# magneano/shyft

Hardware: AMD Instinct MI355X
Metric: cell-steps/sec (cells×timesteps/wall) for pt_gs_k at 1/2/4/8 MI355X (higher is better)
Workload: dtype f64

## Files before the change

shyft_amd/csrc/device/gamma_lean.h:

```cpp
#pragma once
#include <hip/hip_runtime.h>

#include "special.h"

namespace shyft_dev {

__device__ __forceinline__ double exp_fast(double x, const gsb_k& k) {
    double r = gsb_exp(x, k);
    if (!(__builtin_fabs(x) <= 708.0)) r = dexp(x);
    return r;
}
__device__ __forceinline__ double log_fast(double x, const gsb_k& k) {
    double r = gsb_log(x, k);
    if (!(x >= 2.2250738585072014e-308 && x <= 1.7976931348623157e308)) r = dlog(x);
    return r;
}

__device__ __forceinline__ gamma_p_result gsb_gamma_pq(double a, double x, double lga, double eps, double ap1,
                                                       const gsb_k& k, bool& ok) {
    const double lx = gsb_log(x, k);
    const double arg = a * lx - x - lga;
    ok = a > 0.0 && x >= 2.2250738585072014e-308 && x <= 1.7976931348623157e308 && __builtin_fabs(arg) <= 708.0;
    const double prefix = gsb_exp(arg, k);
    gamma_p_result r;
    r.prefix = prefix;
    r.p = r.p1 = 0.0;
    if (!ok) return r;
    if (x < ap1) {
        double ap = a, E = 1.0, B = 0.0, xn = 1.0;
        for (int n = 1; n <= 2000; ++n) {
            ap = ap + 1.0;
            xn = xn * x;
            E = E * ap;
            B = __builtin_fma(B, ap, xn);
            if (xn < eps * (B + E)) break;
        }
        ok = ok && E <= detmath::GPQ_SCALE_HI;
        const double aE = a * E;
        const double pp = prefix * ((B + E) / aE);
        const double pp1 = prefix * (B / aE);
        r.p = pp < 1.0 ? pp : 1.0;
        r.p1 = pp1 < 1.0 ? pp1 : 1.0;
    } else {
        double bcf = x + 1.0 - a;
        double Pm = 1.0, Qm = 0.0, P = bcf, Qd = 1.0, di = 0.0, bigP = 0.0;
        for (int i = 1; i <= 2000; ++i) {
            di = di + 1.0;
            const double an = -di * (di - a);
            bcf = bcf + 2.0;
            const double Pn = __builtin_fma(bcf, P, an * Pm);
            const double Qn = __builtin_fma(bcf, Qd, an * Qm);
            const double cross = Pn * Qd;
            const double diff = cross - P * Qn;
            Pm = P; Qm = Qd;
            P = Pn; Qd = Qn;
            if (__builtin_fabs(diff) <= eps * __builtin_fabs(cross)) break;
            bigP = __builtin_fmax(bigP, __builtin_fabs(P));
        }
        ok = ok && !(bigP > detmath::GPQ_SCALE_HI);
        const double q = prefix * (Qd / P);
        const double q1 = q + prefix / a;
        const double pp = 1.0 - q;
        const double pp1 = 1.0 - q1;
        r.p = pp > 0.0 ? pp : 0.0;
        r.p1 = pp1 > 0.0 ? pp1 : 0.0;
    }
    return r;
}

__device__ __noinline__ gamma_p_result gs_gamma_pq_general(double a, double x, double lga) {
    return gamma_p_prefix(a, x, lga, detmath::gamma_snow_policy_eps(a));
}

}
```

shyft_amd/csrc/device/ptgsk_dev.h:

```cpp
#pragma once
#include <hip/hip_runtime.h>
#include <stdint.h>

#include "pt_dev.h"
#include "special.h"
#include "gamma_lean.h"
#include "../include_internal/layout.h"


namespace shyft_dev {

constexpr double GS_TOL = 1.0e-10;

struct gs_state {
    double albedo, lwc, surface_heat, alpha, sdc_melt_mean, acc_melt, iso_pot_energy, temp_swe;
};

struct lgamma_cache {
    double a = -1.0, v = 0.0;
    __device__ inline double get(double shape) {
        if (shape != a) { a = shape; v = dlgamma(shape); }
        return v;
    }
    __device__ inline double job_lgamma(double shape) { return get(shape); }
};
template <bool DEFER_JOB = false>
struct lgamma_cache_lds {
    double* a;
    double* v;
    __device__ inline double get(double shape) {
        const int t = threadIdx.x;
        if (shape != a[t]) { a[t] = shape; v[t] = dlgamma(shape); }
        return v[t];
    }
    __device__ inline double job_lgamma(double shape) {
        if (!DEFER_JOB) return get(shape);
        a[threadIdx.x] = shape;
        return __builtin_nan("");
    }
};

struct gs_lw {
    double p = __builtin_nan(""), p1 = __builtin_nan("");
};

__device__ __forceinline__ gamma_p_result gs_gamma_pq_cs(double a, double x, double lga) {
    const gsb_k k = gsb_load();
    bool ok;
    gamma_p_result r = gsb_gamma_pq(a, x, lga, detmath::gamma_snow_policy_eps(a), a + 1.0, k, ok);
    if (!ok) r = gs_gamma_pq_general(a, x, lga);
    return r;
}

template <class LGC>
__device__ inline void calc_snow_state(double shape, double scale, double y0, double lambda, double lwd,
                                       double max_water_frac, double temp_swe, double& swe, double& sca,
                                       LGC& lgc, gs_lw& lw) {
    lw.p = lw.p1 = __builtin_nan("");
    double y = 0.0, y1 = 0.0;
    const double m = shape * scale;
    if (lambda <= 0.0) {
        swe = m;
        sca = 1.0 - y0;
    } else if (lambda / scale > 1.3 * shape + 20.0) {
        swe = sca = 0.0;
        return;
    } else {
        const double x = lambda / scale;
        const gamma_p_result g = gs_gamma_pq_cs(shape, x, lgc.get(shape));
        y = g.p;
        y1 = y - g.prefix / shape;
        swe = m * (1.0 - y1) - lambda * (1 - y);
        sca = (1.0 - y) * (1.0 - y0);
    }
    if (lwd > m)
        swe *= 1.0 + max_water_frac;
    else if (lwd > 0.0) {
        const double sat = lwd / max_water_frac;
        const double x = sat / scale;
        const gamma_p_result g = gs_gamma_pq_cs(shape, x, lgc.get(shape));
        lw.p = g.p;
        lw.p1 = g.p1;
        const double ssa = g.p;
        const double ssa1 = ssa - g.prefix / shape;
        const double liqwat = max_water_frac * (m * (ssa1 - y1) + sat * (1.0 - ssa) - lambda * (1.0 - y));
        swe += liqwat;
    }
    swe += temp_swe;
    swe *= 1.0 - y0;
}

__device__ inline double gs_calc_q(double a, double b, double z, double lga) {
    const gamma_p_result g = gs_gamma_pq(a, z / b, lga);
    return a * b * g.p1 + z * (1.0 - g.p);
}


#ifdef SHYFT_PROF
#define SHYFT_PROF_NF , int& nf_evals
#else
#define SHYFT_PROF_NF
#endif
__device__ __noinline__ double gs_corr_lwc(double z1, double a1, double b1, double a2, double b2,
                                           double q1, double lga2 SHYFT_PROF_NF) {
#ifdef SHYFT_ABLATE_BRENT
    return z1 * 0.5;
#endif
    const double Q1 = q1 == q1 ? q1 : gs_calc_q(a1, b1, z1, dlgamma(a1));
    auto f = [&](double z) {
#ifdef SHYFT_PROF
        ++nf_evals;
#endif
        const double v = gs_calc_q(a2, b2, z, lga2) - Q1;
        return v * v;
    };
    double min = 0.0, max = z1;
    const double tolerance = 0x1p-11;
    const double golden = (double)0.3819660f;
    double x, w, v, u, delta, delta2, fu, fv, fw, fx, mid, fract1, fract2;
    x = w = v = max;
    fw = fv = fx = f(x);
    delta2 = delta = 0;
    int count = 60;
    do {
        mid = (min + max) / 2;
        fract1 = tolerance * fabs(x) + tolerance / 4;
        fract2 = 2 * fract1;
        if (fabs(x - mid) <= (fract2 - (max - min) / 2)) break;
        if (fabs(delta2) > fract1) {
            double r = (x - w) * (fx - fv);
            double q = (x - v) * (fx - fw);
            double p = (x - v) * q - (x - w) * r;
            q = 2 * (q - r);
            if (q > 0) p = -p;
            q = fabs(q);
            double td = delta2;
            delta2 = delta;
            if ((fabs(p) >= fabs(q * td / 2)) || (p <= q * (min - x)) || (p >= q * (max - x))) {
                delta2 = (x >= mid) ? min - x : max - x;
                delta = golden * delta2;
            } else {
                delta = p / q;
                u = x + delta;
                if (((u - min) < fract2) || ((max - u) < fract2)) delta = (mid - x) < 0 ? -fabs(fract1) : fabs(fract1);
            }
        } else {
            delta2 = (x >= mid) ? min - x : max - x;
            delta = golden * delta2;
        }
        u = (fabs(delta) >= fract1) ? (x + delta) : (delta > 0 ? x + fabs(fract1) : x - fabs(fract1));
        fu = f(u);
        if (fu <= fx) {
            if (u >= x) min = x; else max = x;
            v = w; w = x; x = u;
            fv = fw; fw = fx; fx = fu;
        } else {
            if (u < x) min = u; else max = u;
            if ((fu <= fw) || (w == x)) {
                v = w; w = u; fv = fw; fw = fu;
            } else if ((fu <= fv) || (v == x) || (v == w)) {
                v = u; fv = fu;
            }
        }
    } while (--count);
    return x;
}

struct gs_cell {
    double forest_fraction, altitude;
    double cv2;
    double inv_cv2;
};

struct gs_mid {
    bool done;
    bool need;
    double snow, rain, potential_melt, start_storage, sdc_scale;
};

struct gs_carry {
    double storage = 0.0;
    gs_lw lw;
    bool ok = false;
};

template <class LGC, class Enqueue, class NewShape>
__device__ inline void gs_front(gs_state& s, gs_mid& m, bool start_melt, double dt_s, double dt_us,
                                      const double* __restrict__ P, const gs_cell& cc, double T, double rad,
                                      double prec_mm_h, double wind_speed, double rel_hum, LGC& lgc,
                                      const gs_carry& carry, Enqueue&& enqueue, NewShape&& new_shape) {
    m.need = false;
    m.done = false;
    double sdc_melt_mean = s.sdc_melt_mean;
    double acc_melt = s.acc_melt;
    double iso_pot_energy = s.iso_pot_energy;
    const double prec = (prec_mm_h * dt_us) / 3600000000.0;
    if (start_melt) acc_melt = iso_pot_energy = 0.0;
    double snow, rain;
    if (T < P[PK_TX]) { snow = prec; rain = 0.0; }
    else { snow = 0.0; rain = prec; }
    if (snow < GS_TOL && sdc_melt_mean < GS_TOL && acc_melt < 0.0) {
        m.done = true;
        return;
    }
    double albedo = s.albedo;
    double lwc = s.lwc;
    double surface_heat = s.surface_heat;
    double alpha = s.alpha;
    const double temp_swe = s.temp_swe;
    double sca = 0.0, storage = 0.0;
    const double min_albedo = P[PK_MIN_ALBEDO];
    const double max_albedo = P[PK_MAX_ALBEDO];
    const double ibgf = P[PK_IBGF];
    const double max_water = P[PK_MAX_WATER];

    const double T_k = T + 273.15;
    const double turb = P[PK_WIND_SCALE] * wind_speed + P[PK_WIND_CONST];
    double vapour_pressure = 33.864 * (dpow8(7.38e-3 * T + 0.8072) - 1.9e-5 * fabs(1.8 * T + 48.0) + 1.316e-3) * rel_hum;
    if (T < 0.0) vapour_pressure *= 1.0 + 9.72e-3 * T + 4.2e-5 * T * T;

    if (snow > GS_TOL)
        albedo += snow * P[PK_ALBEDO_RANGE] / P[PK_SNOWFALL_RESET];
    else {
        if (T < 0.0) albedo -= P[PK_SLOW_DECAY];
        else albedo = min_albedo + P[PK_FAST_DECAY] * (albedo - min_albedo);
    }
    albedo = smax(smin(albedo, max_albedo), min_albedo);

    const double sigma = 5.670373e-8;
    double effect = rad * (1.0 - albedo);
    const dexp_pair gse = dexp2(6.87e-2 * dlog(vapour_pressure / T_k), 0.103 * T - 0.186);
    effect += 0.98 * sigma * gse.a * dpow4(T_k);
    if (T > 0.0 && snow < GS_TOL) effect += rain * T * 4180.0 / dt_s;
    if (T <= 0.0 && rain < GS_TOL) effect += snow * T * 2050.0 / dt_s;

    if (P[PK_ISO] != 0.0) {
        const double iso_effect = effect - P[PK_BB0] + turb * (T + 1.7 * (vapour_pressure - 6.12));
        iso_pot_energy += iso_effect * dt_s / 333660.0;
    }
    const double sst = smin(0.0, 1.16 * T - 2.09);
    if (sst > -GS_TOL)
        effect += turb * (T + 1.7 * (vapour_pressure - 6.12)) - P[PK_BB0];
    else
        effect += turb * (T - sst + 1.7 * (vapour_pressure - 6.132 * gse.b)) -
                  0.98 * sigma * dpow4(sst + 273.15);

    double delta_sh = -surface_heat;
    surface_heat = P[PK_SURFACE_MAG] * 2050.0 * sst * 0.5;
    delta_sh += surface_heat;
    double energy = effect * dt_s;
    if (delta_sh > 0.0) energy -= delta_sh;
    const double potential_melt = smax(0.0, energy / 333660.0);

    double sdc_scale = sdc_melt_mean / alpha;
    gs_lw lw;
    if (carry.ok && !start_melt) {
        storage = carry.storage;
        lw = carry.lw;
    } else {
        calc_snow_state(alpha, sdc_scale, ibgf, acc_melt, lwc, max_water, temp_swe, storage, sca, lgc, lw);
    }
    m.start_storage = storage;

    if (acc_melt < 0.0) {
        if (snow < GS_TOL) snow = 0.0;
        else {
            const double alpha_prev = alpha;
            const double sdc_scale_prev = sdc_scale;
            const double sdc_snow = snow / (1.0 - ibgf);
            alpha = (sdc_melt_mean * alpha + sdc_snow / cc.cv2) / (sdc_snow + sdc_melt_mean);
            sdc_melt_mean += sdc_snow;
            sdc_scale = sdc_melt_mean / alpha;
            if (lwc > 0.0 && sdc_snow > 0.01 * sdc_melt_mean) {
                m.need = true;
                const double z1 = lwc / max_water;
                const double a1 = alpha_prev;
                const double b1 = sdc_scale_prev > 0.0 ? sdc_scale_prev : sdc_scale;
                const double q1 = (sdc_scale_prev > 0.0 && lw.p == lw.p) ? a1 * b1 * lw.p1 + z1 * (1.0 - lw.p)
                                                                          : __builtin_nan("");
                enqueue(z1, a1, b1, alpha, sdc_scale, q1, lgc.job_lgamma(alpha));
            }
        }
        if (!(sdc_melt_mean <= potential_melt)) {
            double lwc_end = lwc + rain;
            double shape = alpha;
            if (potential_melt > 0.0) {
                lwc_end += potential_melt;
                shape = smax(0.1, (sdc_melt_mean - potential_melt) / sdc_scale);
                if (shape > cc.inv_cv2) shape = cc.inv_cv2;
            }
            if (m.need || lwc_end > 0.0) new_shape(shape);
        }
    }
    (void)sca;
    m.snow = snow;
    m.rain = rain;
    m.potential_melt = potential_melt;
    m.sdc_scale = sdc_scale;
    s.albedo = albedo;
    s.surface_heat = surface_heat;
    s.iso_pot_energy = iso_pot_energy;
    s.alpha = alpha;
    s.sdc_melt_mean = sdc_melt_mean;
    s.acc_melt = acc_melt;
}

template <class LGC, class Enqueue>
__device__ inline void gs_front(gs_state& s, gs_mid& m, bool start_melt, double dt_s, double dt_us,
                                      const double* __restrict__ P, const gs_cell& cc, double T, double rad,
                                      double prec_mm_h, double wind_speed, double rel_hum, LGC& lgc,
                                      const gs_carry& carry, Enqueue&& enqueue) {
    gs_front(s, m, start_melt, dt_s, dt_us, P, cc, T, rad, prec_mm_h, wind_speed, rel_hum, lgc, carry, enqueue,
             [](double) {});
}

template <class LGC>
__device__ inline void gs_back(gs_state& s, const gs_mid& m, double z, double& r_sca, double& r_storage,
                                     double& r_outflow, bool snow_season, double dt_us, const double* __restrict__ P,
                                     const gs_cell& cc, double prec_mm_h, LGC& lgc, gs_carry& carry) {
    if (m.done) {
        carry.ok = false;
        carry.storage = 0.0;
        carry.lw = gs_lw();
        s.albedo = P[PK_MAX_ALBEDO];
        s.surface_heat = 0.0;
        s.iso_pot_energy = 0.0;
        r_sca = 0.0;
        r_storage = 0.0;
        r_outflow = prec_mm_h;
        return;
    }
    const double ibgf = P[PK_IBGF];
    const double max_water = P[PK_MAX_WATER];
    const double prec = (prec_mm_h * dt_us) / 3600000000.0;
    double snow = m.snow;
    const double rain = m.rain;
    double lwc = s.lwc, alpha = s.alpha, temp_swe = s.temp_swe, sca = 0.0;
    double storage = m.start_storage;
    double sdc_melt_mean = s.sdc_melt_mean, acc_melt = s.acc_melt, potential_melt = m.potential_melt;
    double sdc_scale = m.sdc_scale;
    if (acc_melt < 0.0) {
        if (m.need) lwc = z * max_water;
        lwc += rain;
        if (sdc_melt_mean <= potential_melt) {
            storage = 0.0;
            sca = sdc_melt_mean = 0.0;
            alpha = P[PK_INV_CV2_PARAM];
            temp_swe = lwc = 0.0;
            acc_melt = -1.0;
            sdc_scale = 0.0;
        } else if (potential_melt > 0.0) {
            sdc_melt_mean -= potential_melt;
            lwc += potential_melt;
            alpha = smax(0.1, sdc_melt_mean / sdc_scale);
            if (alpha > cc.inv_cv2) alpha = cc.inv_cv2;
            sdc_scale = sdc_melt_mean / alpha;
        }
    } else {
        temp_swe += snow / (1.0 - ibgf);
        if (temp_swe > 0.0) {
            const double melt = smin(temp_swe, potential_melt);
            temp_swe -= melt;
            potential_melt -= melt;
            lwc += melt;
            if (temp_swe < GS_TOL) temp_swe = 0.0;
        }
        acc_melt += potential_melt;
        lwc += rain + potential_melt;
        if (P[PK_ISO] == 0.0 || snow_season) {
            if (storage < smax(0.2, 2 * temp_swe) || storage < 0.2 * rain) {
                storage += snow;
                if (storage > GS_TOL) {
                    sca = 1.0 - ibgf;
                    sdc_melt_mean = storage / sca;
                } else {
                    sca = sdc_melt_mean = 0.0;
                }
                alpha = P[PK_INV_CV2_PARAM];
                temp_swe = lwc = 0.0;
                acc_melt = -1.0;
                sdc_scale = sdc_melt_mean / alpha;
            }
        }
    }
    calc_snow_state(alpha, sdc_scale, ibgf, acc_melt, lwc, max_water, temp_swe, storage, sca, lgc, carry.lw);
    carry.storage = storage;
    carry.ok = true;
    double outflow = prec + m.start_storage - storage;
    if (outflow < 0.0) outflow = 0.0;

    s.lwc = lwc;
    s.alpha = alpha;
    s.sdc_melt_mean = sdc_melt_mean;
    s.acc_melt = acc_melt;
    s.temp_swe = temp_swe;
    r_sca = sca;
    r_storage = storage;
    r_outflow = (outflow * 3600000000.0) / dt_us;
}

__device__ inline double kirchner_f(double ln_q, double p_minus_e, double c1, double c2, double c3) {
    const dexp_pair ge = dexp2(c1 + c2 * ln_q + c3 * ln_q * ln_q, -ln_q);
    return ge.a >= 1.e-30 ? ge.a * (p_minus_e * ge.b - 1.0) : 0.0;
}

template <bool INL = false>
__device__ inline bool kirchner_step(double& q, double& q_avg, double p, double e, double t1, double c1, double c2,
                                     double c3) {
    const double abs_err = 1.0e-7, rel_err = 1.0e-8;
    if (q < 0.00001) q = 0.00001;
#ifdef SHYFT_ABLATE_KIRCHNER
    q_avg = q; q = q + 0.01 * (p - e); return true;
#endif
    const double pe = p - e;
    const kmath<INL> km;
    auto kirchner_f = [&](double ln_q, double p_minus_e, double c1_, double c2_, double c3_) {
        const dexp_pair ge = km.exp2(c1_ + c2_ * ln_q + c3_ * ln_q * ln_q, -ln_q);
        return ge.a >= 1.e-30 ? ge.a * (p_minus_e * ge.b - 1.0) : 0.0;
    };
    auto dexp = [&](double v) { return km.exp(v); };
    auto dlog = [&](double v) { return km.log(v); };
    double x = dlog(q);
    double dxdt = kirchner_f(x, pe, c1, c2, c3);
    double t = 0.0, dt = t1;
    double x_old = x, dxdt_old = dxdt, t_old = 0.0;
    double k3 = 0, k4 = 0, k5 = 0, k6 = 0;
    double area = 0.0, f_a = q, t_a = 0.0;
    int attempts = 0;
    bool ok = true;
    const double b21 = 1.0 / 5;
    const double b31 = 3.0 / 40, b32 = 9.0 / 40;
    const double b41 = 44.0 / 45, b42 = -56.0 / 15, b43 = 32.0 / 9;
    const double b51 = 19372.0 / 6561, b52 = -25360.0 / 2187, b53 = 64448.0 / 6561, b54 = -212.0 / 729;
    const double b61 = 9017.0 / 3168, b62 = -355.0 / 33, b63 = 46732.0 / 5247, b64 = 49.0 / 176, b65 = -5103.0 / 18656;
    const double c1_ = 35.0 / 384, c3_ = 500.0 / 1113, c4_ = 125.0 / 192, c5_ = -2187.0 / 6784, c6_ = 11.0 / 84;
    const double dc1 = c1_ - 5179.0 / 57600, dc3 = c3_ - 7571.0 / 16695, dc4 = c4_ - 393.0 / 640,
                 dc5 = c5_ - -92097.0 / 339200, dc6 = c6_ - 187.0 / 2100, dc7 = -1.0 / 40;
    auto attempt = [&](const double h) -> bool {
        double xt = 1.0 * x + h * b21 * dxdt;
        const double k2 = kirchner_f(xt, pe, c1, c2, c3);
        xt = 1.0 * x + h * b31 * dxdt + h * b32 * k2;
        const double s3 = kirchner_f(xt, pe, c1, c2, c3);
        xt = 1.0 * x + h * b41 * dxdt + h * b42 * k2 + h * b43 * s3;
        const double s4 = kirchner_f(xt, pe, c1, c2, c3);
        xt = 1.0 * x + h * b51 * dxdt + h * b52 * k2 + h * b53 * s3 + h * b54 * s4;
        const double s5 = kirchner_f(xt, pe, c1, c2, c3);
        xt = 1.0 * x + h * b61 * dxdt + h * b62 * k2 + h * b63 * s3 + h * b64 * s4 + h * b65 * s5;
        const double s6 = kirchner_f(xt, pe, c1, c2, c3);
        const double xo = 1.0 * x + h * c1_ * dxdt + h * c3_ * s3 + h * c4_ * s4 + h * c5_ * s5 + h * c6_ * s6;
        const double dxdt_o = kirchner_f(xo, pe, c1, c2, c3);
        const double xerr = h * dc1 * dxdt + h * dc3 * s3 + h * dc4 * s4 + h * dc5 * s5 + h * dc6 * s6 + h * dc7 * dxdt_o;
        const double err = fabs(xerr) / (abs_err + rel_err * (1.0 * fabs(x) + 1.0 * h * fabs(dxdt)));
        if (err > 1.0) {
            dt = h * smax(0.9 * dexp(-1.0 / 3.0 * dlog(err)), 1.0 / 5.0);
            return ++attempts < 500;
        }
        attempts = 0;
        t_old = t;
        t = t + h;
        dt = h;
        if (err < 0.5 && t < t1) {
            const double e2 = smax(0.00032, err);
            dt = h * (9.0 / 10.0 * dexp(-1.0 / 5.0 * dlog(e2)));
        }
        x_old = x; dxdt_old = dxdt;
        x = xo; dxdt = dxdt_o;
        k3 = s3; k4 = s4; k5 = s5; k6 = s6;
        if (t < t1) {
            const double fv = dexp(x);
            area += 0.5 * (f_a + fv) * (t - t_a);
            f_a = fv;
            t_a = t;
// ... 48 lines not shown
```

shyft_amd/csrc/kernels/ptgsk.hip:

```cpp
#include <hip/hip_runtime.h>
#include <stdint.h>
#include <stdlib.h>

#include "../device/ptgsk_dev.h"
#include "../device/gs_brent.h"
#include "../device/stream.h"
#include "../device/wave_place.h"
#include "../include_internal/kernels.h"
#include "../../../include/shyft_hip.h"

using namespace shyft_dev;

#define GS_BRENT_JOB gs_corr_lwc_lean

#ifdef SHYFT_PROF
__device__ unsigned long long g_ptgsk_prof[12];
extern "C" int shyft_ptgsk_prof_read(unsigned long long* out) {
    if (hipMemcpyFromSymbol(out, HIP_SYMBOL(g_ptgsk_prof), sizeof(g_ptgsk_prof)) != hipSuccess) return 1;
    unsigned long long z[12] = {};
    return hipMemcpyToSymbol(HIP_SYMBOL(g_ptgsk_prof), z, sizeof z) != hipSuccess;
}
#define PROF_DECL unsigned long long prof_acc[6] = {0, 0, 0, 0, 0, 0}, prof_lg = 0; unsigned long long prof_t = __builtin_amdgcn_s_memtime();
#define PROF_MARK(k) do { const unsigned long long t_ = __builtin_amdgcn_s_memtime(); prof_acc[k] += t_ - prof_t; prof_t = t_; } while (0)
#define PROF_FLUSH() do { if ((threadIdx.x & 63) == 0) { for (int k_ = 0; k_ < 6; ++k_) atomicAdd(&g_ptgsk_prof[k_], prof_acc[k_]); atomicAdd(&g_ptgsk_prof[11], prof_lg); } } while (0)
#else
#define PROF_DECL
#define PROF_MARK(k) ((void)0)
#define PROF_FLUSH() ((void)0)
#endif

namespace {

#ifndef SHYFT_PTGSK_NT
#define SHYFT_PTGSK_NT 1
#endif
constexpr bool STREAM_NT = SHYFT_PTGSK_NT != 0;

constexpr int BLOCK = 256;

#ifndef SHYFT_LB_WAVES
#define SHYFT_LB_WAVES 4
#endif

#ifndef SHYFT_PTGSK_LEAN
#define SHYFT_PTGSK_LEAN 1
#endif

constexpr int BRENT_PRIO = 3;

#ifndef SHYFT_PTGSK_LGQ
#define SHYFT_PTGSK_LGQ 1
#endif
#ifndef SHYFT_PTGSK_LGQ_NOBRENT
#define SHYFT_PTGSK_LGQ_NOBRENT 0
#endif
#ifndef SHYFT_PTGSK_LGQ_JOBLG
#define SHYFT_PTGSK_LGQ_JOBLG 1
#endif

#ifndef SHYFT_PTGSK_BOPEN
#define SHYFT_PTGSK_BOPEN 2
#endif

template <bool COMPACT, bool UNIFORM, bool ENS = false, int WAVES = SHYFT_LB_WAVES, int B = BLOCK, bool SPEC = false,
          bool LEAN = false>
__global__ __launch_bounds__(B, WAVES) void ptgsk_run_kernel(const ptgsk_kargs a) {
    static_assert(COMPACT, "the Brent jobs always go through the workgroup queue");
    const int cell = blockIdx.x * blockDim.x + threadIdx.x;
    bool valid = cell < a.n_cells;
    if (valid && a.active && !a.active[cell]) valid = false;
    const int lc = valid ? cell : 0;
    const size_t N = (size_t)a.n_cells;
    const size_t NF = ENS ? (size_t)a.f_cols : N;
    const size_t fcl = ENS ? (size_t)a.fcol[lc] : (size_t)lc;
    const double* __restrict__ Pg = UNIFORM ? a.params : a.params + (size_t)a.set_ix[lc] * PTGSK_NP;
    __shared__ double lpar[UNIFORM ? PTGSK_NP : 1];
    if (UNIFORM && threadIdx.x < PTGSK_NP) lpar[threadIdx.x] = a.params[threadIdx.x];
    const double* __restrict__ P = UNIFORM ? (const double*)lpar : Pg;

    const double* __restrict__ cc = a.cellc;
    gs_cell gcell;
    gcell.forest_fraction = cc[PC_FOREST * N + lc];
    gcell.altitude = cc[PC_ALTITUDE * N + lc];
    gcell.cv2 = cc[PC_CV2 * N + lc];
    gcell.inv_cv2 = cc[PC_INV_CV2 * N + lc];
    __shared__ double lcc[11][B];
    {
        const int t = threadIdx.x;
        lcc[0][t] = gcell.forest_fraction;
        lcc[1][t] = gcell.altitude;
        lcc[2][t] = gcell.cv2;
        lcc[3][t] = gcell.inv_cv2;
        lcc[4][t] = cc[PC_GLACIER * N + lc];
        lcc[5][t] = cc[PC_SNOW_STORAGE * N + lc];
        lcc[6][t] = cc[PC_KIRCHNER_ROUTED_PREC * N + lc];
        lcc[7][t] = cc[PC_DIRECT_RESPONSE * N + lc];
        lcc[8][t] = cc[PC_AREA * N + lc];
    }
#define glacier_fraction (lcc[4][threadIdx.x])
#define snow_storage_fraction (lcc[5][threadIdx.x])
#define kirchner_routed_prec (lcc[6][threadIdx.x])
#define direct_response_fraction (lcc[7][threadIdx.x])
#define kirchner_fraction (1 - lcc[7][threadIdx.x])
#define cell_area_m2 (lcc[8][threadIdx.x])
#define glacier_area_m2 (lcc[8][threadIdx.x] * lcc[4][threadIdx.x])
#define LOAD_GCELL()                                   \
    do {                                               \
        gcell.forest_fraction = lcc[0][threadIdx.x];   \
        gcell.altitude = lcc[1][threadIdx.x];          \
        gcell.cv2 = lcc[2][threadIdx.x];               \
        gcell.inv_cv2 = lcc[3][threadIdx.x];           \
    } while (0)

    const double mmh_to_m3s_scale_factor = 1 / (3600.0 * 1000.0);

    double* __restrict__ st = a.state;
    gs_state s;
    s.albedo = st[PS_ALBEDO * N + lc];
    s.lwc = st[PS_LWC * N + lc];
    s.surface_heat = st[PS_SURFACE_HEAT * N + lc];
    s.alpha = st[PS_ALPHA * N + lc];
    s.sdc_melt_mean = st[PS_SDC_MELT_MEAN * N + lc];
    s.acc_melt = st[PS_ACC_MELT * N + lc];
    s.iso_pot_energy = st[PS_ISO_POT_ENERGY * N + lc];
    s.temp_swe = st[PS_TEMP_SWE * N + lc];
    double q = st[PS_KIRCHNER_Q * N + lc];
    lcc[9][threadIdx.x] = -1.0;
    lcc[10][threadIdx.x] = 0.0;
    constexpr bool LGQ = SHYFT_PTGSK_LGQ != 0 && B == 256 && !SPEC;
    constexpr bool JOBLG = LGQ && SHYFT_PTGSK_LGQ_JOBLG != 0;
    constexpr int BOPEN = (B == 256 && !SPEC) ? SHYFT_PTGSK_BOPEN : 0;
    lgamma_cache_lds<JOBLG> lgc{lcc[9], lcc[10]};
    gs_carry carry;
    int32_t err = 0;

    const size_t TW = (size_t)a.win_len;
    const double* __restrict__ f_temp = a.forcing + (size_t)FV_TEMPERATURE * TW * NF;
    const double* __restrict__ f_prec = a.forcing + (size_t)FV_PRECIPITATION * TW * NF;
    const double* __restrict__ f_ws = a.forcing + (size_t)FV_WIND_SPEED * TW * NF;
    const double* __restrict__ f_rh = a.forcing + (size_t)FV_REL_HUM * TW * NF;
    const double* __restrict__ f_rad = a.forcing + (size_t)FV_RADIATION * TW * NF;
    double* __restrict__ R = a.resp;
    const size_t RS = TW * N;
    double* __restrict__ SS = LEAN ? nullptr : a.state_series;
    const size_t SSS = (TW + 1) * N;
    const int wed = (int)Pg[PK_WED];
    const int64_t snow_lo = (int64_t)((int)(Pg[PK_WED] * 24) - (int)(Pg[PK_NWD] * 24)) * 3600000000LL;
    const int64_t snow_hi = (int64_t)(int)(Pg[PK_WED] * 24) * 3600000000LL;

    __shared__ double jq[SPEC ? 1 : GSQ_ROWS][SPEC ? 1 : B];
    __shared__ double sz1[SPEC ? B : 1], sa1[SPEC ? B : 1], sb1[SPEC ? B : 1], sa2[SPEC ? B : 1], sb2[SPEC ? B : 1],
        sq1[SPEC ? B : 1], slg2[SPEC ? B : 1], sres[SPEC ? B : 1];
    double* const jz1 = SPEC ? sz1 : jq[GSQ_Z1];
    double* const ja1 = SPEC ? sa1 : jq[GSQ_A1];
    double* const jb1 = SPEC ? sb1 : jq[GSQ_B1];
    double* const ja2 = SPEC ? sa2 : jq[GSQ_A2];
    double* const jb2 = SPEC ? sb2 : jq[GSQ_B2];
    double* const jq1 = SPEC ? sq1 : jq[GSQ_Q1];
    double* const jlg2 = SPEC ? slg2 : jq[GSQ_LG2];
    double* const jres = SPEC ? sres : jq[GSQ_RES];
    __shared__ double jsz[SPEC ? 64 : 1], jsf[SPEC ? 64 : 1];
    __shared__ int jcount[2];
    __shared__ unsigned short lq[LGQ ? B : 1];
    __shared__ unsigned short jown[JOBLG ? B : 1];
    __shared__ int lcount[2];
    __shared__ int wsimd[B / 64];
    publish_wave_simd(wsimd);
    if (COMPACT) {
        if (threadIdx.x == 0) {
            jcount[0] = jcount[1] = 0;
            if (LGQ) lcount[0] = lcount[1] = 0;
        }
        __syncthreads();
    }
    const int jrot = solver_lane0<B>(wsimd);

    auto collect_state = [&](size_t wi) {
        SS[0 * SSS + wi * N + cell] = cell_area_m2 * q * mmh_to_m3s_scale_factor;
        SS[1 * SSS + wi * N + cell] = s.albedo;
        SS[2 * SSS + wi * N + cell] = s.lwc * snow_storage_fraction;
        SS[3 * SSS + wi * N + cell] = s.surface_heat;
        SS[4 * SSS + wi * N + cell] = s.alpha;
        SS[5 * SSS + wi * N + cell] = s.sdc_melt_mean;
        SS[6 * SSS + wi * N + cell] = s.acc_melt;
        SS[7 * SSS + wi * N + cell] = s.iso_pot_energy;
        SS[8 * SSS + wi * N + cell] = s.temp_swe * snow_storage_fraction;
    };

    const int i_end = a.step0 + a.n_steps;
    PROF_DECL
    for (int i = a.step0; i < i_end; ++i) {
        const double gm_direct = P[PK_GM_DIRECT];
        const double gm_routed = 1 - gm_direct;
        const double dtf = P[PK_DTF];
        const double p_corr = P[PK_PCORR];
        const double kc1 = P[PK_C1], kc2 = P[PK_C2], kc3 = P[PK_C3];
        const size_t wi = (size_t)(i - a.win0);
        const size_t fo = wi * N + lc;
        const size_t ff = ENS ? wi * NF + fcl : fo;
        double temp = 0, rad = 0, rel_hum = 0, prec = 0, wind_speed = 0;
        if (valid) {
            temp = stream_ld<STREAM_NT && !ENS>(&f_temp[ff]);
            rad = stream_ld<STREAM_NT && !ENS>(&f_rad[ff]);
            rel_hum = stream_ld<STREAM_NT && !ENS>(&f_rh[ff]);
            prec = stream_ld<STREAM_NT && !ENS>(&f_prec[ff]) * p_corr;
            wind_speed = stream_ld<STREAM_NT && !ENS>(&f_ws[ff]);
            if (SS) collect_state(wi);
        }
        const bool start_melt = a.doy[i] == wed;
        const int64_t trel = a.t_rel_year_us[i];
        const bool snow_season = trel >= snow_lo && trel < snow_hi;

        gs_mid m;
        m.need = false;
        m.done = true;
        LOAD_GCELL();
        if (threadIdx.x == 0) {
            jcount[(i + 1) & 1] = 0;
            if (LGQ) lcount[(i + 1) & 1] = 0;
        }
        int slot = -1;
        bool queued = false;
        auto new_shape = [&](double shape) {
            if (LGQ && shape != lcc[9][threadIdx.x]) {
                lq[atomicAdd(&lcount[i & 1], 1)] = (unsigned short)threadIdx.x;
                lcc[9][threadIdx.x] = shape;
                queued = true;
            }
        };
        auto brent_jobs = [&](int t, int nj) {
            if (JOBLG)
                for (int j = t; j < nj; j += B) {
                    const double lga2 = dlgamma(ja2[j]);
                    jlg2[j] = lga2;
                    const int o = jown[j];
                    if (lcc[9][o] == ja2[j]) lcc[10][o] = lga2;
                }
            if (BOPEN) {
                __builtin_amdgcn_fence(__ATOMIC_ACQ_REL, "wavefront");
                const int L = gs_brent_group<BOPEN>(nj);
                for (int tt = t; tt < L * nj; tt += B) gs_brent_job_open<B>((gsq_lds*)&jq[0][0], tt, L);
                return;
            }
            for (int j = t; j < nj; j += B)
                jres[j] = GS_BRENT_JOB(jz1[j], ja1[j], jb1[j], ja2[j], jb2[j], jq1[j], jlg2[j]);
        };
        auto lgamma_jobs = [&](int first, int stride, int nl) {
            for (int j = first; j < nl; j += stride) {
                const int o = lq[j];
                lcc[10][o] = dlgamma(lcc[9][o]);
            }
        };
        auto enqueue = [&](double z1, double a1, double b1, double a2, double b2, double q1, double lga2) {
            slot = atomicAdd(&jcount[i & 1], 1);
            jz1[slot] = z1; ja1[slot] = a1; jb1[slot] = b1; ja2[slot] = a2; jb2[slot] = b2;
            jq1[slot] = q1; jlg2[slot] = lga2;
            if (JOBLG) jown[slot] = (unsigned short)threadIdx.x;
        };
#ifndef SHYFT_ABLATE_SNOW
        if (valid)
            gs_front(s, m, start_melt, a.dt_s, a.dt_us, P, gcell, temp, rad, prec, wind_speed, rel_hum, lgc, carry, enqueue,
                     new_shape);
#endif
        PROF_MARK(0);
        double z = 0.0;
        {
            __syncthreads();
            PROF_MARK(1);
            const int nj = jcount[i & 1];
            const int nl = LGQ ? lcount[i & 1] : 0;
            auto lgamma_phase = [&](int t) {
                const int ns = (nj + 63) & ~63;
                if (ns >= B) lgamma_jobs(t, B, nl);
                else if (t >= ns) lgamma_jobs(t - ns, B - ns, nl);
            };
            if (nj > 0) {
#ifdef SHYFT_PROF
                const unsigned long long tb = __builtin_amdgcn_s_memtime();
                if (threadIdx.x < nj) __builtin_amdgcn_s_setprio(BRENT_PRIO);
                brent_jobs((int)threadIdx.x, nj);
                __builtin_amdgcn_s_setprio(0);
                if (threadIdx.x < nj && (threadIdx.x & 63) == 0)
                    atomicAdd(&g_ptgsk_prof[8], (unsigned long long)(__builtin_amdgcn_s_memtime() - tb));
                if (LGQ && nl > 0) {
                    const unsigned long long tl = __builtin_amdgcn_s_memtime();
                    lgamma_phase((int)threadIdx.x);
                    prof_lg += __builtin_amdgcn_s_memtime() - tl;
                }
#else
                const int t = SPEC ? (int)threadIdx.x : (int)((threadIdx.x - jrot) & (B - 1));
                if (t < nj) __builtin_amdgcn_s_setprio(BRENT_PRIO);
                const int L = SPEC ? (4 * nj <= 64 ? 4 : 2 * nj <= 64 ? 2 : 0) : 0;
                if (L) {
                    const int jj = L == 4 ? t >> 2 : t >> 1;
                    if (t < 64 && jj < nj) {
                        const gsb_zf r = gs_corr_lwc_spec(jz1[jj], ja1[jj], jb1[jj], ja2[jj], jb2[jj], jq1[jj], jlg2[jj], t & (L - 1));
                        jsz[t] = r.z;
                        jsf[t] = r.f;
                    }
                    __syncthreads();
                    if (t < nj) {
                        gsb_memo mm;
#pragma unroll
                        for (int k = 0; k < 4; ++k) {
                            const int e = L * t + (k < L ? k : 0);
                            mm.z[k] = jsz[e];
                            mm.f[k] = jsf[e];
                        }
                        jres[t] = gs_corr_lwc_memo(jz1[t], ja1[t], jb1[t], ja2[t], jb2[t], jq1[t], jlg2[t], mm);
                    }
                } else {
                    brent_jobs(t, nj);
                }
                __builtin_amdgcn_s_setprio(0);
                if (LGQ && nl > 0) lgamma_phase(t);
#endif
                __syncthreads();
                if (!LEAN && a.read_delay > 0 && (threadIdx.x >> 6) != 0)
                    for (int k = 0; k < a.read_delay; ++k) __builtin_amdgcn_s_sleep(127);
                if (slot >= 0) z = jres[slot];
            } else if (LGQ && SHYFT_PTGSK_LGQ_NOBRENT > 0 && nl >= SHYFT_PTGSK_LGQ_NOBRENT) {
                lgamma_jobs((int)threadIdx.x, B, nl);
                __syncthreads();
            } else if (LGQ && queued) {
                lcc[10][threadIdx.x] = dlgamma(lcc[9][threadIdx.x]);
            }
        }
        PROF_MARK(2);
        if (!valid) {
            carry = gs_carry();
            continue;
        }
        double gs_sca, gs_storage, gs_outflow;
        LOAD_GCELL();
#ifdef SHYFT_ABLATE_SNOW
        gs_sca = 0.0; gs_storage = 0.0; gs_outflow = prec + 0.0 * z;
#else
        gs_back(s, m, z, gs_sca, gs_storage, gs_outflow, snow_season, a.dt_us, P, gcell, prec, lgc, carry);
#endif
        PROF_MARK(3);

        const double sca_area = cell_area_m2 * gs_sca;
        double gm_melt_m3s = 0.0;
        if (!(glacier_area_m2 <= sca_area || temp <= 0.0))
            gm_melt_m3s = dtf * temp * (glacier_area_m2 - sca_area) * (0.001 / 86400.0);
        double ae_exp;
        const double pot_evap =
            pt_pot_evap_exp<true>(P[PK_PT_ALBEDO], P[PK_PT_ALPHA], temp, rad, rel_hum, -q * 3.0 / P[PK_AE_SCALE], ae_exp) *
            3600.0;
        const double ae = pot_evap * (1.0 - ae_exp) * (1.0 - smax(gs_sca, glacier_fraction));
        const double gm_mmh = gm_melt_m3s / (mmh_to_m3s_scale_factor * cell_area_m2);
        PROF_MARK(4);
        double q_avg;
        if (!kirchner_step<true>(q, q_avg, gs_outflow * snow_storage_fraction + prec * kirchner_routed_prec + gm_routed * gm_mmh,
                           ae, a.t1_hours, kc1, kc2, kc3))
            err = ERR_KIRCHNER_MAX_ITER;
        const double total_discharge = smax(0.0, prec - ae) * direct_response_fraction + gm_direct * gm_mmh +
                                       q_avg * kirchner_fraction;
        const double charge_m3s = +(cell_area_m2 * prec * mmh_to_m3s_scale_factor) -
                                  (cell_area_m2 * ae * mmh_to_m3s_scale_factor) + gm_melt_m3s -
                                  (cell_area_m2 * total_discharge * mmh_to_m3s_scale_factor);
        stream_st<STREAM_NT>(&R[0 * RS + fo], cell_area_m2 * total_discharge * mmh_to_m3s_scale_factor);
        stream_st<STREAM_NT>(&R[1 * RS + fo], charge_m3s);
        if (!LEAN && a.collect >= 1) {
            R[2 * RS + fo] = gs_sca;
            R[3 * RS + fo] = gs_storage * snow_storage_fraction;
        }
        if (!LEAN && a.collect >= 2) {
            R[4 * RS + fo] = cell_area_m2 * (gs_outflow * snow_storage_fraction) * mmh_to_m3s_scale_factor;
            R[5 * RS + fo] = gm_melt_m3s;
            R[6 * RS + fo] = ae;
            R[7 * RS + fo] = pot_evap;
        }
        if (SS && i + 1 == i_end) collect_state(wi + 1);
        PROF_MARK(5);
    }
    PROF_FLUSH();
    if (!valid) return;
    st[PS_ALBEDO * N + cell] = s.albedo;
    st[PS_LWC * N + cell] = s.lwc;
    st[PS_SURFACE_HEAT * N + cell] = s.surface_heat;
    st[PS_ALPHA * N + cell] = s.alpha;
    st[PS_SDC_MELT_MEAN * N + cell] = s.sdc_melt_mean;
    st[PS_ACC_MELT * N + cell] = s.acc_melt;
    st[PS_ISO_POT_ENERGY * N + cell] = s.iso_pot_energy;
    st[PS_TEMP_SWE * N + cell] = s.temp_swe;
    st[PS_KIRCHNER_Q * N + cell] = q;
    if (err) a.err[cell] = err;
}
#undef LOAD_GCELL
#undef glacier_fraction
#undef snow_storage_fraction
#undef kirchner_routed_prec
#undef direct_response_fraction
#undef kirchner_fraction
#undef cell_area_m2
#undef glacier_area_m2

#ifndef SHYFT_PTGSK_BUDGET_WAVES
#define SHYFT_PTGSK_BUDGET_WAVES 7
#endif
constexpr int ST_BOPEN = SHYFT_PTGSK_BOPEN ? SHYFT_PTGSK_BOPEN : 2;
__global__ __launch_bounds__(256, SHYFT_PTGSK_BUDGET_WAVES) void ptgsk_callee_budget_kernel(const ptgsk_kargs a) {
    if (a.n_cells >= 0) return;
    const int c = threadIdx.x;
    gs_state s{};
    gs_mid m{};
    lgamma_cache lgc;
    gs_carry carry;
    gs_cell gc{};
    double q = a.dt_s, qa = 0.0, sca, sto, outf;
    double j[7] = {};
    gs_front(s, m, c == 0, a.dt_s, a.dt_us, a.params, gc, q, q, q, q, q, lgc, carry,
             [&](double z1, double a1, double b1, double a2, double b2, double q1, double lga2) {
                 j[0] = z1; j[1] = a1; j[2] = b1; j[3] = a2; j[4] = b2; j[5] = q1; j[6] = lga2;
             });
    double z = gs_corr_lwc_lean(j[0], j[1], j[2], j[3], j[4], j[5], j[6]);
    __shared__ double jq[GSQ_ROWS][BLOCK];
    for (int r = 0; r < 7; ++r) jq[r][c] = j[r];
    gs_brent_job_open<BLOCK>((gsq_lds*)&jq[0][0], c, 4);
    z += jq[GSQ_RES][c];
    gs_back(s, m, z, sca, sto, outf, c == 1, a.dt_us, a.params, gc, q, lgc, carry);
    double e;
    const double pe = pt_pot_evap_exp<true>(0.2, 1.26, q, q, q, q, e);
    kirchner_step<true>(q, qa, outf, pe * e, a.t1_hours, -2.4, 0.9, -0.1);
    a.resp[c] = q + qa + sca + sto + s.lwc;
}

constexpr int ST_BLOCK = 256;

__global__ __launch_bounds__(ST_BLOCK, SHYFT_PTGSK_BUDGET_WAVES) void ptgsk_st_explog_inline_kernel(
    const double* __restrict__ in, size_t n, double* __restrict__ out) {
    const size_t i = blockIdx.x * (size_t)ST_BLOCK + threadIdx.x;
    if (i >= n) return;
    const kmath<true> km;
    const double x = in[i];
    out[i] = km.exp(x);
    out[n + i] = km.log(x);
}

__global__ __launch_bounds__(ST_BLOCK, SHYFT_PTGSK_BUDGET_WAVES) void ptgsk_st_explog_pairs_kernel(
    const double* __restrict__ in, size_t n, double* __restrict__ out) {
    const size_t i = blockIdx.x * (size_t)ST_BLOCK + threadIdx.x;
    if (i >= n) return;
    const kmath<true> km;
    const double x = in[i], y = in[n + i];
    const dexp_pair e = km.exp2(x, y);
    const dexp_pair l = km.log2p(x, y);
    out[i] = e.a;
    out[n + i] = e.b;
    out[2 * n + i] = l.a;
    out[3 * n + i] = l.b;
}

__global__ __launch_bounds__(ST_BLOCK, SHYFT_PTGSK_BUDGET_WAVES) void ptgsk_st_explog_calls_kernel(
    const double* __restrict__ in, size_t n, double* __restrict__ out) {
    const size_t i = blockIdx.x * (size_t)ST_BLOCK + threadIdx.x;
    if (i >= n) return;
    const double x = in[i], y = in[n + i];
    out[i] = dexp(x);
    out[n + i] = dlog(x);
    const dexp_pair e = dexp2(x, y);
    out[2 * n + i] = e.a;
    out[3 * n + i] = e.b;
}

__global__ __launch_bounds__(ST_BLOCK, SHYFT_PTGSK_BUDGET_WAVES) void ptgsk_st_powers_kernel(
    const double* __restrict__ in, size_t n, double* __restrict__ out) {
    const size_t i = blockIdx.x * (size_t)ST_BLOCK + threadIdx.x;
    if (i >= n) return;
    const double x = in[i], y = in[n + i];
    out[i] = dpowr(x, y);
    out[n + i] = dpow4(x);
    out[2 * n + i] = dpow8(x);
    out[3 * n + i] = dpow(x, y);
}

__global__ __launch_bounds__(ST_BLOCK, SHYFT_PTGSK_BUDGET_WAVES) void ptgsk_st_gamma_kernel(
    const double* __restrict__ in, size_t n, double* __restrict__ out) {
    const size_t i = blockIdx.x * (size_t)ST_BLOCK + threadIdx.x;
    if (i >= n) return;
    const double a = in[i], x = in[n + i];
    const double lga = dlgamma(a);
    bool ok;
    (void)gsb_gamma_pq(a, x, lga, detmath::gamma_snow_policy_eps(a), a + 1.0, gsb_load(), ok);
    const gamma_p_result r = gs_gamma_pq_cs(a, x, lga);
    out[i] = r.p;
    out[n + i] = r.p1;
    out[2 * n + i] = r.prefix;
    out[3 * n + i] = ok ? 1.0 : 0.0;
}

__device__ __forceinline__ double st_brent_q1(double mode, double z1, double a1, double b1) {
    return mode != 0.0 ? gs_calc_q(a1, b1, z1, dlgamma(a1)) : __builtin_nan("");
}

__global__ __launch_bounds__(ST_BLOCK, SHYFT_PTGSK_BUDGET_WAVES) void ptgsk_st_brent_kernel(
    const double* __restrict__ in, size_t n, double* __restrict__ out) {
    const size_t i = blockIdx.x * (size_t)ST_BLOCK + threadIdx.x;
    if (i >= n) return;
    const double z1 = in[i], a1 = in[n + i], b1 = in[2 * n + i], a2 = in[3 * n + i], b2 = in[4 * n + i];
    const double q1 = st_brent_q1(in[5 * n + i], z1, a1, b1);
    const double lga2 = dlgamma(a2);
#ifdef SHYFT_PROF
    int nf_evals = 0;
    out[i] = gs_corr_lwc(z1, a1, b1, a2, b2, q1, lga2, nf_evals);
#else
    out[i] = gs_corr_lwc(z1, a1, b1, a2, b2, q1, lga2);
#endif
    out[n + i] = GS_BRENT_JOB(z1, a1, b1, a2, b2, q1, lga2);
}

template <int L>
__global__ __launch_bounds__(64, 2) void ptgsk_st_brent_spec_kernel(const double* __restrict__ in, size_t n,
                                                                    double* __restrict__ out) {
    static_assert(L == 4 || L == 2, "4 or 2 point lanes per job");
    constexpr int JOBS = 64 / L;
    __shared__ double jz1[JOBS], ja1[JOBS], jb1[JOBS], ja2[JOBS], jb2[JOBS], jq1[JOBS], jlg2[JOBS];
    __shared__ double jsz[64], jsf[64];
    const int t = threadIdx.x;
    const size_t j0 = blockIdx.x * (size_t)JOBS;
    const int nj = n - j0 < (size_t)JOBS ? (int)(n - j0) : JOBS;
    if (t < nj) {
        const size_t i = j0 + t;
        jz1[t] = in[i]; ja1[t] = in[n + i]; jb1[t] = in[2 * n + i]; ja2[t] = in[3 * n + i]; jb2[t] = in[4 * n + i];
        jq1[t] = st_brent_q1(in[5 * n + i], jz1[t], ja1[t], jb1[t]);
        jlg2[t] = dlgamma(ja2[t]);
    }
    __syncthreads();
    const int jj = L == 4 ? t >> 2 : t >> 1;
    if (t < 64 && jj < nj) {
        const gsb_zf r = gs_corr_lwc_spec(jz1[jj], ja1[jj], jb1[jj], ja2[jj], jb2[jj], jq1[jj], jlg2[jj], t & (L - 1));
        jsz[t] = r.z;
        jsf[t] = r.f;
    }
    __syncthreads();
    if (t < nj) {
        gsb_memo mm;
#pragma unroll
        for (int k = 0; k < 4; ++k) {
            const int e = L * t + (k < L ? k : 0);
            mm.z[k] = jsz[e];
            mm.f[k] = jsf[e];
        }
        out[j0 + t] = gs_corr_lwc_memo(jz1[t], ja1[t], jb1[t], ja2[t], jb2[t], jq1[t], jlg2[t], mm);
    }
}

template <int JOBS>
__global__ __launch_bounds__(ST_BLOCK, SHYFT_PTGSK_BUDGET_WAVES) void ptgsk_st_brent_open_kernel(
    const double* __restrict__ in, size_t n, double* __restrict__ out) {
    static_assert(JOBS == 16 || JOBS == 32, "16 or 32 jobs per workgroup");
    __shared__ double jq[GSQ_ROWS][ST_BLOCK];
    const int t = threadIdx.x;
    const size_t j0 = blockIdx.x * (size_t)JOBS;
    const int nj = n - j0 < (size_t)JOBS ? (int)(n - j0) : JOBS;
    if (t < nj) {
        const size_t i = j0 + t;
        jq[GSQ_Z1][t] = in[i]; jq[GSQ_A1][t] = in[n + i]; jq[GSQ_B1][t] = in[2 * n + i];
        jq[GSQ_A2][t] = in[3 * n + i]; jq[GSQ_B2][t] = in[4 * n + i];
        jq[GSQ_Q1][t] = st_brent_q1(in[5 * n + i], jq[GSQ_Z1][t], jq[GSQ_A1][t], jq[GSQ_B1][t]);
        jq[GSQ_LG2][t] = dlgamma(jq[GSQ_A2][t]);
    }
    __syncthreads();
    const int L = gs_brent_group<ST_BOPEN>(nj);
    if (t < L * nj) gs_brent_job_open<ST_BLOCK>((gsq_lds*)&jq[0][0], t, L);
    __syncthreads();
    if (t < nj) out[j0 + t] = jq[GSQ_RES][t];
}

}


hipError_t launch_ptgsk_run(const ptgsk_kargs& a, hipStream_t stream) {
    const int grid = (a.n_cells + BLOCK - 1) / BLOCK;
    if (grid == 0) return hipSuccess;
    int n_cu = 256;
    {
        int dev = 0;
        if (hipGetDevice(&dev) == hipSuccess) {
            int v = 0;
            if (hipDeviceGetAttribute(&v, hipDeviceAttributeMultiprocessorCount, dev) == hipSuccess && v > 0) n_cu = v;
        }
    }
    static const char* force = getenv("SHYFT_PTGSK_WAVES");
    const bool small = a.instance ? a.instance == 2 : force ? force[0] == '2' : grid <= 2 * n_cu;
    const bool lean = SHYFT_PTGSK_LEAN && a.collect == 0 && !a.state_series && a.read_delay == 0;
    if (a.n_cells < 0)
        hipLaunchKernelGGL(ptgsk_callee_budget_kernel, dim3(1), dim3(BLOCK), 0, stream, a);
    if (a.fcol) {
        hipLaunchKernelGGL((ptgsk_run_kernel<true, false, true>), dim3(grid), dim3(BLOCK), 0, stream, a);
    } else if (small) {
        const int g64 = (a.n_cells + 63) / 64;
        if (lean) {
            if (a.uniform_params) hipLaunchKernelGGL((ptgsk_run_kernel<true, true, false, 2, 64, true, true>), dim3(g64), dim3(64), 0, stream, a);
            else hipLaunchKernelGGL((ptgsk_run_kernel<true, false, false, 2, 64, true, true>), dim3(g64), dim3(64), 0, stream, a);
        } else if (a.uniform_params) hipLaunchKernelGGL((ptgsk_run_kernel<true, true, false, 2, 64, true>), dim3(g64), dim3(64), 0, stream, a);
        else hipLaunchKernelGGL((ptgsk_run_kernel<true, false, false, 2, 64, true>), dim3(g64), dim3(64), 0, stream, a);
    } else if (lean) {
        if (a.uniform_params) hipLaunchKernelGGL((ptgsk_run_kernel<true, true, false, SHYFT_LB_WAVES, BLOCK, false, true>), dim3(grid), dim3(BLOCK), 0, stream, a);
        else hipLaunchKernelGGL((ptgsk_run_kernel<true, false, false, SHYFT_LB_WAVES, BLOCK, false, true>), dim3(grid), dim3(BLOCK), 0, stream, a);
    } else {
        if (a.uniform_params) hipLaunchKernelGGL((ptgsk_run_kernel<true, true>), dim3(grid), dim3(BLOCK), 0, stream, a);
        else hipLaunchKernelGGL((ptgsk_run_kernel<true, false>), dim3(grid), dim3(BLOCK), 0, stream, a);
    }
    return hipGetLastError();
}

hipError_t launch_ptgsk_selftest(int fn, const double* in, size_t n, double* out, hipStream_t stream) {
    if (n == 0) return hipSuccess;
    const dim3 grid((unsigned)((n + ST_BLOCK - 1) / ST_BLOCK)), block(ST_BLOCK);
    switch (fn) {
        case SHYFT_HIP_DST_EXPLOG_INLINE: hipLaunchKernelGGL(ptgsk_st_explog_inline_kernel, grid, block, 0, stream, in, n, out); break;
        case SHYFT_HIP_DST_EXPLOG_CALLS: hipLaunchKernelGGL(ptgsk_st_explog_calls_kernel, grid, block, 0, stream, in, n, out); break;
        case SHYFT_HIP_DST_EXPLOG_PAIRS: hipLaunchKernelGGL(ptgsk_st_explog_pairs_kernel, grid, block, 0, stream, in, n, out); break;
        case SHYFT_HIP_DST_POWERS: hipLaunchKernelGGL(ptgsk_st_powers_kernel, grid, block, 0, stream, in, n, out); break;
        case SHYFT_HIP_DST_GAMMA_LEAN: hipLaunchKernelGGL(ptgsk_st_gamma_kernel, grid, block, 0, stream, in, n, out); break;
        case SHYFT_HIP_DST_BRENT: hipLaunchKernelGGL(ptgsk_st_brent_kernel, grid, block, 0, stream, in, n, out); break;
        case SHYFT_HIP_DST_BRENT_SPEC4:
            hipLaunchKernelGGL(ptgsk_st_brent_spec_kernel<4>, dim3((unsigned)((n + 15) / 16)), dim3(64), 0, stream, in, n, out);
            break;
        case SHYFT_HIP_DST_BRENT_SPEC2:
            hipLaunchKernelGGL(ptgsk_st_brent_spec_kernel<2>, dim3((unsigned)((n + 31) / 32)), dim3(64), 0, stream, in, n, out);
            break;
        case SHYFT_HIP_DST_BRENT_OPEN4:
            hipLaunchKernelGGL(ptgsk_st_brent_open_kernel<16>, dim3((unsigned)((n + 15) / 16)), block, 0, stream, in, n, out);
            break;
        case SHYFT_HIP_DST_BRENT_OPEN2:
// ... 7 lines not shown
```

Measured before the change: 11.78 billion.

## Hand-write gamma series and continued-fraction loops in asm; drop unused cell fields

Replaces the incomplete-gamma series and continued-fraction loops with inline GCN assembly. Each loop is unrolled by two, uses v_cmpx to mask converged lanes out of exec, and leaves early once every lane has converged, which removes compiler-generated per-iteration exec bookkeeping. It also removes the unused forest_fraction and altitude fields from the per-cell struct and the LDS cache, shrinking the shared array from 11 to 9 rows. The assembly ties the code to this ISA. Because the pair unroll changes the iteration count, odd-count exits must be recovered by parity, and the series loop's iteration cap differs slightly from the original.

After: 12.16 billion (median of 6 runs). 1.03x the previous value.

```diff
diff --git a/shyft_amd/csrc/device/gamma_lean.h b/shyft_amd/csrc/device/gamma_lean.h
--- a/shyft_amd/csrc/device/gamma_lean.h
+++ b/shyft_amd/csrc/device/gamma_lean.h
@@ -16,6 +16,88 @@
     return r;
 }
 
+#ifndef SHYFT_GAMMA_LOOPS
+#define SHYFT_GAMMA_LOOPS 3
+#endif
+
+#if SHYFT_GAMMA_LOOPS
+#define GSB_SERIES_TERM                                 \
+    "v_add_f64 %[ap], %[ap], 1.0\n\t"                   \
+    "v_mul_f64 %[xn], %[x], %[xn]\n\t"                  \
+    "v_mul_f64 %[E], %[E], %[ap]\n\t"                   \
+    "v_fma_f64 %[B], %[B], %[ap], %[xn]\n\t"            \
+    "v_add_f64 %[s], %[E], %[B]\n\t"                    \
+    "v_mul_f64 %[t], %[eps], %[s]\n\t"                  \
+    "v_cmpx_nlt_f64_e32 vcc, %[xn], %[t]\n\t"
+
+__device__ __forceinline__ void gsb_series_loop(double a, double x, double eps, double& E_, double& B_, double& S_) {
+    double ap = a, E = 1.0, B = 0.0, xn = 1.0, s, t;
+    unsigned long long live;
+    unsigned pairs;
+    asm volatile(
+        "s_mov_b64 %[live], exec\n\t"
+        "s_movk_i32 %[pairs], 999\n"
+        ".Lgsb_series_%=:\n\t"
+        GSB_SERIES_TERM
+        "s_cbranch_execz .Lgsb_series_done_%=\n\t"
+        GSB_SERIES_TERM
+        "s_sub_u32 %[pairs], %[pairs], 1\n\t"
+        "s_cbranch_scc1 .Lgsb_series_done_%=\n\t"
+        "s_cbranch_execnz .Lgsb_series_%=\n"
+        ".Lgsb_series_done_%=:\n\t"
+        "s_mov_b64 exec, %[live]"
+        : [ap] "+v"(ap), [xn] "+v"(xn), [E] "+v"(E), [B] "+v"(B), [s] "=&v"(s), [t] "=&v"(t),
+          [live] "=&s"(live), [pairs] "=&s"(pairs)
+        : [x] "v"(x), [eps] "v"(eps)
+        : "vcc", "scc");
+    E_ = E;
+    B_ = B;
+    S_ = s;
+}
+
+#define GSB_CF_TERM(PM, P, QM, QD)                                  \
+    "v_add_f64 %[di], %[di], 1.0\n\t"                               \
+    "v_add_f64 %[t], %[di], -%[a]\n\t"                              \
+    "v_mul_f64 %[t], %[t], -%[di]\n\t"                              \
+    "v_add_f64 %[bcf], %[bcf], 2.0\n\t"                             \
+    "v_mul_f64 %[" PM "], %[t], %[" PM "]\n\t"                      \
+    "v_mul_f64 %[" QM "], %[" QM "], %[t]\n\t"                      \
+    "v_fma_f64 %[" PM "], %[bcf], %[" P "], %[" PM "]\n\t"          \
+    "v_fma_f64 %[" QM "], %[bcf], %[" QD "], %[" QM "]\n\t"         \
+    "v_mul_f64 %[t], %[" QD "], %[" PM "]\n\t"                      \
+    "v_mul_f64 %[u], %[" P "], %[" QM "]\n\t"                       \
+    "v_add_f64 %[u], %[t], -%[u]\n\t"                               \
+    "v_mul_f64 %[t], %[eps], |%[t]|\n\t"                            \
+    "v_cmpx_nle_f64_e64 vcc, |%[u]|, %[t]\n\t"
+
+__device__ __forceinline__ void gsb_cf_loop(double a, double eps, double bcf, double& P_, double& Qd_, double& bigP_) {
+    double pa = 1.0, pb = bcf, qa = 0.0, qb = 1.0, di = 0.0, bigP = 0.0, t, u;
+    unsigned long long live;
+    asm volatile(
+        "s_mov_b64 %[live], exec\n"
+        ".Lgsb_cf_%=:\n\t"
+        GSB_CF_TERM("pa", "pb", "qa", "qb")
+        "s_cbranch_execz .Lgsb_cf_done_%=\n\t"
+        "v_max_f64 %[big], %[big], |%[pa]|\n\t"
+        GSB_CF_TERM("pb", "pa", "qb", "qa")
+        "v_max_f64 %[big], %[big], |%[pb]|\n\t"
+        "v_cmpx_gt_f64_e32 vcc, 2000.0, %[di]\n\t"
+        "s_cbranch_execnz .Lgsb_cf_%=\n"
+        ".Lgsb_cf_done_%=:\n\t"
+        "s_mov_b64 exec, %[live]"
+        : [pa] "+v"(pa), [pb] "+v"(pb), [qa] "+v"(qa), [qb] "+v"(qb), [di] "+v"(di), [bcf] "+v"(bcf),
+          [big] "+v"(bigP), [t] "=&v"(t), [u] "=&v"(u), [live] "=&s"(live)
+        : [a] "v"(a), [eps] "v"(eps)
+        : "vcc");
+    const bool odd = ((int)di & 1) != 0;
+    P_ = odd ? pa : pb;
+    Qd_ = odd ? qa : qb;
+    bigP_ = bigP;
+}
+#undef GSB_SERIES_TERM
+#undef GSB_CF_TERM
+#endif
+
 __device__ __forceinline__ gamma_p_result gsb_gamma_pq(double a, double x, double lga, double eps, double ap1,
                                                        const gsb_k& k, bool& ok) {
     const double lx = gsb_log(x, k);
@@ -27,6 +109,10 @@
     r.p = r.p1 = 0.0;
     if (!ok) return r;
     if (x < ap1) {
+#if SHYFT_GAMMA_LOOPS & 1
+        double E, B, S;
+        gsb_series_loop(a, x, eps, E, B, S);
+#else
         double ap = a, E = 1.0, B = 0.0, xn = 1.0;
         for (int n = 1; n <= 2000; ++n) {
             ap = ap + 1.0;
@@ -35,13 +121,22 @@
             B = __builtin_fma(B, ap, xn);
             if (xn < eps * (B + E)) break;
         }
+#endif
         ok = ok && E <= detmath::GPQ_SCALE_HI;
         const double aE = a * E;
+#if SHYFT_GAMMA_LOOPS & 1
+        const double pp = prefix * (S / aE);
+#else
         const double pp = prefix * ((B + E) / aE);
+#endif
         const double pp1 = prefix * (B / aE);
         r.p = pp < 1.0 ? pp : 1.0;
         r.p1 = pp1 < 1.0 ? pp1 : 1.0;
     } else {
+#if SHYFT_GAMMA_LOOPS & 2
+        double P, Qd, bigP;
+        gsb_cf_loop(a, eps, x + 1.0 - a, P, Qd, bigP);
+#else
         double bcf = x + 1.0 - a;
         double Pm = 1.0, Qm = 0.0, P = bcf, Qd = 1.0, di = 0.0, bigP = 0.0;
         for (int i = 1; i <= 2000; ++i) {
@@ -57,6 +152,7 @@
             if (__builtin_fabs(diff) <= eps * __builtin_fabs(cross)) break;
             bigP = __builtin_fmax(bigP, __builtin_fabs(P));
         }
+#endif
         ok = ok && !(bigP > detmath::GPQ_SCALE_HI);
         const double q = prefix * (Qd / P);
         const double q1 = q + prefix / a;
diff --git a/shyft_amd/csrc/device/ptgsk_dev.h b/shyft_amd/csrc/device/ptgsk_dev.h
--- a/shyft_amd/csrc/device/ptgsk_dev.h
+++ b/shyft_amd/csrc/device/ptgsk_dev.h
@@ -167,7 +167,6 @@
 }
 
 struct gs_cell {
-    double forest_fraction, altitude;
     double cv2;
     double inv_cv2;
 };
diff --git a/shyft_amd/csrc/kernels/ptgsk.hip b/shyft_amd/csrc/kernels/ptgsk.hip
--- a/shyft_amd/csrc/kernels/ptgsk.hip
+++ b/shyft_amd/csrc/kernels/ptgsk.hip
@@ -80,36 +80,30 @@
 
     const double* __restrict__ cc = a.cellc;
     gs_cell gcell;
-    gcell.forest_fraction = cc[PC_FOREST * N + lc];
-    gcell.altitude = cc[PC_ALTITUDE * N + lc];
     gcell.cv2 = cc[PC_CV2 * N + lc];
     gcell.inv_cv2 = cc[PC_INV_CV2 * N + lc];
-    __shared__ double lcc[11][B];
+    __shared__ double lcc[9][B];
     {
         const int t = threadIdx.x;
-        lcc[0][t] = gcell.forest_fraction;
-        lcc[1][t] = gcell.altitude;
-        lcc[2][t] = gcell.cv2;
-        lcc[3][t] = gcell.inv_cv2;
-        lcc[4][t] = cc[PC_GLACIER * N + lc];
-        lcc[5][t] = cc[PC_SNOW_STORAGE * N + lc];
-        lcc[6][t] = cc[PC_KIRCHNER_ROUTED_PREC * N + lc];
-        lcc[7][t] = cc[PC_DIRECT_RESPONSE * N + lc];
-        lcc[8][t] = cc[PC_AREA * N + lc];
-    }
-#define glacier_fraction (lcc[4][threadIdx.x])
-#define snow_storage_fraction (lcc[5][threadIdx.x])
-#define kirchner_routed_prec (lcc[6][threadIdx.x])
-#define direct_response_fraction (lcc[7][threadIdx.x])
-#define kirchner_fraction (1 - lcc[7][threadIdx.x])
-#define cell_area_m2 (lcc[8][threadIdx.x])
-#define glacier_area_m2 (lcc[8][threadIdx.x] * lcc[4][threadIdx.x])
+        lcc[0][t] = gcell.cv2;
+        lcc[1][t] = gcell.inv_cv2;
+        lcc[2][t] = cc[PC_GLACIER * N + lc];
+        lcc[3][t] = cc[PC_SNOW_STORAGE * N + lc];
+        lcc[4][t] = cc[PC_KIRCHNER_ROUTED_PREC * N + lc];
+        lcc[5][t] = cc[PC_DIRECT_RESPONSE * N + lc];
+        lcc[6][t] = cc[PC_AREA * N + lc];
+    }
+#define glacier_fraction (lcc[2][threadIdx.x])
+#define snow_storage_fraction (lcc[3][threadIdx.x])
+#define kirchner_routed_prec (lcc[4][threadIdx.x])
+#define direct_response_fraction (lcc[5][threadIdx.x])
+#define kirchner_fraction (1 - lcc[5][threadIdx.x])
+#define cell_area_m2 (lcc[6][threadIdx.x])
+#define glacier_area_m2 (lcc[6][threadIdx.x] * lcc[2][threadIdx.x])
 #define LOAD_GCELL()                                   \
     do {                                               \
-        gcell.forest_fraction = lcc[0][threadIdx.x];   \
-        gcell.altitude = lcc[1][threadIdx.x];          \
-        gcell.cv2 = lcc[2][threadIdx.x];               \
-        gcell.inv_cv2 = lcc[3][threadIdx.x];           \
+        gcell.cv2 = lcc[0][threadIdx.x];               \
+        gcell.inv_cv2 = lcc[1][threadIdx.x];           \
     } while (0)
 
     const double mmh_to_m3s_scale_factor = 1 / (3600.0 * 1000.0);
@@ -125,12 +119,12 @@
     s.iso_pot_energy = st[PS_ISO_POT_ENERGY * N + lc];
     s.temp_swe = st[PS_TEMP_SWE * N + lc];
     double q = st[PS_KIRCHNER_Q * N + lc];
-    lcc[9][threadIdx.x] = -1.0;
-    lcc[10][threadIdx.x] = 0.0;
+    lcc[7][threadIdx.x] = -1.0;
+    lcc[8][threadIdx.x] = 0.0;
     constexpr bool LGQ = SHYFT_PTGSK_LGQ != 0 && B == 256 && !SPEC;
     constexpr bool JOBLG = LGQ && SHYFT_PTGSK_LGQ_JOBLG != 0;
     constexpr int BOPEN = (B == 256 && !SPEC) ? SHYFT_PTGSK_BOPEN : 0;
-    lgamma_cache_lds<JOBLG> lgc{lcc[9], lcc[10]};
+    lgamma_cache_lds<JOBLG> lgc{lcc[7], lcc[8]};
     gs_carry carry;
     int32_t err = 0;
 
@@ -222,9 +216,9 @@
         int slot = -1;
         bool queued = false;
         auto new_shape = [&](double shape) {
-            if (LGQ && shape != lcc[9][threadIdx.x]) {
+            if (LGQ && shape != lcc[7][threadIdx.x]) {
                 lq[atomicAdd(&lcount[i & 1], 1)] = (unsigned short)threadIdx.x;
-                lcc[9][threadIdx.x] = shape;
+                lcc[7][threadIdx.x] = shape;
                 queued = true;
             }
         };
@@ -234,7 +228,7 @@
                     const double lga2 = dlgamma(ja2[j]);
                     jlg2[j] = lga2;
                     const int o = jown[j];
-                    if (lcc[9][o] == ja2[j]) lcc[10][o] = lga2;
+                    if (lcc[7][o] == ja2[j]) lcc[8][o] = lga2;
                 }
             if (BOPEN) {
                 __builtin_amdgcn_fence(__ATOMIC_ACQ_REL, "wavefront");
@@ -248,7 +242,7 @@
         auto lgamma_jobs = [&](int first, int stride, int nl) {
             for (int j = first; j < nl; j += stride) {
                 const int o = lq[j];
-                lcc[10][o] = dlgamma(lcc[9][o]);
+                lcc[8][o] = dlgamma(lcc[7][o]);
             }
         };
         auto enqueue = [&](double z1, double a1, double b1, double a2, double b2, double q1, double lga2) {
@@ -323,7 +317,7 @@
                 lgamma_jobs((int)threadIdx.x, B, nl);
                 __syncthreads();
             } else if (LGQ && queued) {
-                lcc[10][threadIdx.x] = dlgamma(lcc[9][threadIdx.x]);
+                lcc[8][threadIdx.x] = dlgamma(lcc[7][threadIdx.x]);
             }
         }
         PROF_MARK(2);
```
